# medinammartin3/Safe-Autonomous-Driving-MPC

Measured on NVIDIA B200. Metric: tracking_mpc_qp_solves_per_sec, higher is better.
Workload: dtype f64

## Files before the change

safe-autonomous-driving-mpc_b200/csrc/mpcb_api.cu:

```cuda
#include <cuda_runtime.h>
#include <math.h>
#include <stdio.h>
#include <stdlib.h>
#include <string.h>

#include <algorithm>
#include <new>
#include <type_traits>
#include <vector>

#include "mpcb200.h"
#include "mpcb_solver.cuh"
#include "mpcb_coop.cuh"

namespace mpcb {

#ifndef MPCB_SOLVE_THREADS
#define MPCB_SOLVE_THREADS 128
#endif
#ifndef MPCB_SOLVE_CTAS
#define MPCB_SOLVE_CTAS 2
#endif
#ifndef MPCB_STORE_MASK
#define MPCB_STORE_MASK 7
#endif
constexpr int SOLVE_THREADS = MPCB_SOLVE_THREADS;
using SolveStore = Store<(MPCB_STORE_MASK != 0 ? SOLVE_THREADS : 1), MPCB_STORE_MASK>;
constexpr size_t SOLVE_SMEM = sizeof(double) * SolveStore::SHARED * SOLVE_THREADS;
#ifndef MPCB_CLS_MASK0
#define MPCB_CLS_MASK0 (1u | 2u | 8u | 32u)
#endif
#ifndef MPCB_CLS_MASK1
#define MPCB_CLS_MASK1 (1u | 2u | 4u | 32u)
#endif
#ifndef MPCB_CLS_MASK2
#define MPCB_CLS_MASK2 7u
#endif
template <int NOBS> struct ClsCfg;
template <> struct ClsCfg<0> { typedef Store<SOLVE_THREADS, MPCB_CLS_MASK0, 0> St; };
template <> struct ClsCfg<1> { typedef Store<SOLVE_THREADS, MPCB_CLS_MASK1, 1> St; };
template <> struct ClsCfg<2> { typedef Store<SOLVE_THREADS, MPCB_CLS_MASK2, 2> St; };
constexpr int cmax3(int a, int b, int c) { return a > b ? (a > c ? a : c) : (b > c ? b : c); }
constexpr size_t CLS_SMEM = sizeof(double) * SOLVE_THREADS * cmax3(ClsCfg<0>::St::SHARED, ClsCfg<1>::St::SHARED, ClsCfg<2>::St::SHARED);
constexpr int CLS_HDR = 4;
constexpr int EVAL_THREADS = 128;

struct SolveIO {
  const double* x0; const double* obs_sv; const int* n_obs;
  double* U; double* Xpred; double* obj; int* status; int* iters; double* cmin; unsigned long long* active;
  double* u0;
  const int* idx;
  const int* n_idx;
  int accumulate;
  const double* U_start;
  int shift_start;
  int n_total;
};

template <bool FIRST_PASS>
__device__ __forceinline__ bool finalize(const DevTable& T, const DevParams& P, const Problem& pb, const SolveOut& so, int b,
                                         bool accumulate, const SolveIO& io, int* __restrict__ fb_list,
                                         int* __restrict__ fb_count) {
  double* __restrict__ U_out = io.U;
  double* __restrict__ Xpred_out = io.Xpred;
  double* __restrict__ obj_out = io.obj;
  int* __restrict__ status_out = io.status;
  int* __restrict__ iters_out = io.iters;
// ... 97 lines not shown
  Problem pb;
  if (live) {
#pragma unroll
    for (int c = 0; c < 5; ++c) pb.x0[c] = io.x0[(size_t)b * 5 + c];
#pragma unroll
    for (int k = 0; k < 2; ++k) { pb.obs[k][0] = io.obs_sv[(size_t)b * 4 + 2 * k]; pb.obs[k][1] = io.obs_sv[(size_t)b * 4 + 2 * k + 1]; }
    pb.n_obs = min(max(io.n_obs[b], 0), 2);
  } else {
#pragma unroll
    for (int c = 0; c < 5; ++c) pb.x0[c] = 0.0;
    pb.obs[0][0] = pb.obs[0][1] = pb.obs[1][0] = pb.obs[1][1] = 0.0;
    pb.n_obs = 0;
  }
  extern __shared__ double solve_smem[];
  double solve_local[SolveStore::LOCAL > 0 ? SolveStore::LOCAL : 1];
  const SolveStore st(solve_smem + threadIdx.x, solve_local);
  SolveOut so = solve_one<FIRST_PASS>(T, P, pb, st, live);
  if (!live) return;
  finalize<FIRST_PASS>(T, P, pb, so, b, io.accumulate != 0, io, fb_list, fb_count);
}

__global__ void __launch_bounds__(256)
mpcb_classify_kernel(int B, const int* __restrict__ idx, const int* __restrict__ n_idx, const int* __restrict__ n_obs,
                     int* __restrict__ cls) {
  const int n_work = idx ? min(*n_idx, B) : B;
  const int t = blockIdx.x * blockDim.x + threadIdx.x;
  const bool live = t < n_work;
  const int b = live ? (idx ? idx[t] : t) : 0;
  const int c = live ? min(max(n_obs[b], 0), 2) : -1;
  const unsigned lane = threadIdx.x & 31u;
#pragma unroll
  for (int k = 0; k < 3; ++k) {
    const unsigned m = __ballot_sync(0xffffffffu, c == k);
    if (m == 0u) continue;
    int base = 0;
    const int leader = __ffs(m) - 1;
    if ((int)lane == leader) base = atomicAdd(cls + k, __popc(m));
    base = __shfl_sync(0xffffffffu, base, leader);
    if (c == k) {
      const int slot = base + __popc(m & ((1u << lane) - 1u));
      MPCB_ASSERT(slot >= 0 && slot < B && b >= 0 && b < B);
      cls[CLS_HDR + (size_t)k * B + slot] = b;
    }
  }
}

__device__ __forceinline__ void load_hot_start(const SolveIO& io, int b, double (&Uh)[NV]) {
  const double* __restrict__ src = io.U_start + (size_t)b * NV;
#pragma unroll
  for (int i = 0; i < NV; ++i) Uh[i] = io.shift_start ? src[i + 2 < NV ? i + 2 : i] : src[i];
}

template <int NOBS>
__device__ __forceinline__ void solve_cls_body(const DevTable& T, const DevParams& P, const SolveIO& io, const int* __restrict__ list,
                                               int n_work, int t0, int* __restrict__ fb_list, int* __restrict__ fb_count) {
  typedef typename ClsCfg<NOBS>::St St;
  const int t = t0 + threadIdx.x;
  const bool live = t < n_work;
  const int b = live ? list[t] : 0;
  MPCB_ASSERT(b >= 0 && b < io.n_total);
  Problem pb;
  if (live) {
#pragma unroll
    for (int c = 0; c < 5; ++c) pb.x0[c] = io.x0[(size_t)b * 5 + c];
#pragma unroll
    for (int k = 0; k < 2; ++k) {
      pb.obs[k][0] = (k < NOBS) ? io.obs_sv[(size_t)b * 4 + 2 * k] : 0.0;
      pb.obs[k][1] = (k < NOBS) ? io.obs_sv[(size_t)b * 4 + 2 * k + 1] : 0.0;
    }
    pb.n_obs = NOBS;
  } else {
#pragma unroll
    for (int c = 0; c < 5; ++c) pb.x0[c] = 0.0;
    pb.obs[0][0] = pb.obs[0][1] = pb.obs[1][0] = pb.obs[1][1] = 0.0;
    pb.n_obs = 0;
  }
  extern __shared__ double solve_smem[];
  double solve_local[St::LOCAL];
  const St st(solve_smem + threadIdx.x, solve_local);
  double Uh[NV];
  const bool hot = io.U_start != nullptr;
  if (hot && live) load_hot_start(io, b, Uh);
  SolveOut so = solve_one<true>(T, P, pb, st, live, (hot && live) ? Uh : nullptr);
  if (!live) return;
  finalize<true>(T, P, pb, so, b, io.accumulate != 0, io, fb_list, fb_count);
}

__global__ void __launch_bounds__(SOLVE_THREADS, MPCB_SOLVE_CTAS)
mpcb_solve_cls_kernel(const __grid_constant__ DevTable T, const __grid_constant__ DevParams P, int B,
                      const __grid_constant__ SolveIO io, const int* __restrict__ cls, int* __restrict__ fb_list,
                      int* __restrict__ fb_count) {
  const int n2 = cls[2], n1 = cls[1], n0 = cls[0];
  const int c2 = (n2 + SOLVE_THREADS - 1) / SOLVE_THREADS, c1 = (n1 + SOLVE_THREADS - 1) / SOLVE_THREADS,
            c0 = (n0 + SOLVE_THREADS - 1) / SOLVE_THREADS;
  int blk = blockIdx.x;
  if (blk < c2) { solve_cls_body<2>(T, P, io, cls + CLS_HDR + (size_t)2 * B, n2, blk * SOLVE_THREADS, fb_list, fb_count); return; }
  blk -= c2;
  if (blk < c1) { solve_cls_body<1>(T, P, io, cls + CLS_HDR + (size_t)1 * B, n1, blk * SOLVE_THREADS, fb_list, fb_count); return; }
  blk -= c1;
  if (blk < c0) solve_cls_body<0>(T, P, io, cls + CLS_HDR, n0, blk * SOLVE_THREADS, fb_list, fb_count);
}

constexpr int COOP_WARPS = 4;
#ifndef MPCB_COOP_CTAS
#define MPCB_COOP_CTAS 2
#endif
constexpr int COOP_CTAS = MPCB_COOP_CTAS;
constexpr int FB_HDR = 4;
constexpr size_t COOP_SMEM = sizeof(WarpShared) * COOP_WARPS;

template <bool FIRST_PASS>
__global__ void __launch_bounds__(COOP_WARPS * 32, COOP_CTAS)
mpcb_coop_kernel(const __grid_constant__ DevTable T, const __grid_constant__ DevParams P, int B,
                 const __grid_constant__ SolveIO io, int* __restrict__ fb_list, int* __restrict__ fb_count,
                 int* __restrict__ cursor) {
  extern __shared__ double coop_smem[];
  const int lane = threadIdx.x & 31, wid = threadIdx.x >> 5;
  WarpShared& ws = reinterpret_cast<WarpShared*>(coop_smem)[wid];
  const int* __restrict__ idx = io.idx;
  const int n_work = idx ? min(*io.n_idx, B) : B;
  for (;;) {
    int t = 0;
    if (lane == 0) t = atomicAdd(cursor, 1);
// ... 274 lines not shown
  c->device = device;
  c->n_sm = prop.multiProcessorCount;
  c->params = *p;
  c->dp = dp;
  const int K = t->K;
  c->K = K;
  c->Ku = t->Ku;
  auto fail = [&](int code) { mpcb_destroy(c); return code; };
  if (cudaMalloc(&c->d_s, sizeof(double) * K) != cudaSuccess) return fail(cuda_fail(cudaGetLastError(), "cudaMalloc"));
  if (cudaMalloc(&c->d_y, sizeof(double) * K * 4) != cudaSuccess) return fail(cuda_fail(cudaGetLastError(), "cudaMalloc"));
  if (cudaMalloc(&c->d_u, sizeof(double) * c->Ku * 2) != cudaSuccess) return fail(cuda_fail(cudaGetLastError(), "cudaMalloc"));
  cudaError_t e;
  if ((e = cudaMemcpy(c->d_s, t->s.data(), sizeof(double) * K, cudaMemcpyHostToDevice)) != cudaSuccess) return fail(cuda_fail(e, "cudaMemcpy"));
  if ((e = cudaMemcpy(c->d_y, t->y.data(), sizeof(double) * K * 4, cudaMemcpyHostToDevice)) != cudaSuccess) return fail(cuda_fail(e, "cudaMemcpy"));
  if ((e = cudaMemcpy(c->d_u, t->u.data(), sizeof(double) * c->Ku * 2, cudaMemcpyHostToDevice)) != cudaSuccess) return fail(cuda_fail(e, "cudaMemcpy"));
  int prio_lo = 0, prio_hi = 0;
  cudaDeviceGetStreamPriorityRange(&prio_lo, &prio_hi);
  if ((e = cudaStreamCreateWithPriority(&c->stream, cudaStreamNonBlocking, prio_hi)) != cudaSuccess) return fail(cuda_fail(e, "cudaStreamCreate"));
  if ((e = cudaEventCreate(&c->ev0)) != cudaSuccess) return fail(cuda_fail(e, "cudaEventCreate"));
  if ((e = cudaEventCreate(&c->ev1)) != cudaSuccess) return fail(cuda_fail(e, "cudaEventCreate"));
  if ((e = cudaEventCreate(&c->ev_mid)) != cudaSuccess) return fail(cuda_fail(e, "cudaEventCreate"));
  if ((e = cudaEventCreateWithFlags(&c->ev_fork, cudaEventDisableTiming)) != cudaSuccess) return fail(cuda_fail(e, "cudaEventCreate"));
  if ((e = cudaFuncSetAttribute(mpcb_solve_cls_kernel, cudaFuncAttributeMaxDynamicSharedMemorySize, (int)CLS_SMEM)) != cudaSuccess ||
      (e = cudaFuncSetAttribute(mpcb_solve_kernel<false>, cudaFuncAttributeMaxDynamicSharedMemorySize, (int)SOLVE_SMEM)) != cudaSuccess ||
      (e = cudaFuncSetAttribute(mpcb_coop_kernel<true>, cudaFuncAttributeMaxDynamicSharedMemorySize, (int)COOP_SMEM)) != cudaSuccess ||
      (e = cudaFuncSetAttribute(mpcb_coop_kernel<false>, cudaFuncAttributeMaxDynamicSharedMemorySize, (int)COOP_SMEM)) != cudaSuccess)
    return fail(cuda_fail(e, "cudaFuncSetAttribute"));
  c->xs[0] = c->stream;
  for (int k = 1; k < 4; ++k) {
    if ((e = cudaStreamCreateWithPriority(&c->xs[k], cudaStreamNonBlocking, std::min(prio_lo, prio_hi + k))) != cudaSuccess) return fail(cuda_fail(e, "cudaStreamCreate"));
    if ((e = cudaEventCreateWithFlags(&c->xe[k], cudaEventDisableTiming)) != cudaSuccess) return fail(cuda_fail(e, "cudaEventCreate"));
  }
  c->dt.s = c->d_s; c->dt.y = c->d_y; c->dt.u = c->d_u;
  c->dt.K = K; c->dt.Ku = c->Ku; c->dt.s_max = t->s_max;
  {
    const int n = 4096;
    const double s0 = t->s[0], span = t->s[K - 1] - t->s[0];
    std::vector<int> lut(n);
    const double scale = span > 0 ? (double)n / span : 0.0;
    for (int b = 0; b < n; ++b) {
      const double edge = s0 + (scale > 0 ? (double)b / scale : 0.0);
      const int lo = (int)(std::lower_bound(t->s.begin(), t->s.end(), edge) - t->s.begin());
      lut[b] = std::min(std::max(lo, 1), K - 1);
    }
    if (cudaMalloc(&c->d_lut, sizeof(int) * n) != cudaSuccess) return fail(cuda_fail(cudaGetLastError(), "cudaMalloc"));
    if ((e = cudaMemcpy(c->d_lut, lut.data(), sizeof(int) * n, cudaMemcpyHostToDevice)) != cudaSuccess) return fail(cuda_fail(e, "cudaMemcpy"));
// ... 4 lines not shown
    if ((e = cudaMemcpy(c->d_sinv, sinv.data(), sizeof(double) * K, cudaMemcpyHostToDevice)) != cudaSuccess) return fail(cuda_fail(e, "cudaMemcpy"));
    c->dt.sinv = c->d_sinv;
  }
  for (int k = 0; k < 4; ++k) c->dt.last[k] = t->last_row[1 + k];
  *out = c;
  return MPCB_OK;
}

int mpcb_destroy(mpcb_handle h) {
  if (!h) return MPCB_ERR_INVALID;
  cudaSetDevice(h->device);
  if (h->d_s) cudaFree(h->d_s);
  if (h->d_y) cudaFree(h->d_y);
  if (h->d_u) cudaFree(h->d_u);
  if (h->d_lut) cudaFree(h->d_lut);
  if (h->d_sinv) cudaFree(h->d_sinv);
  for (int k = 0; k < 2; ++k) {
    if (h->gslot[k].exec) cudaGraphExecDestroy(h->gslot[k].exec);
    if (h->gslot[k].graph) cudaGraphDestroy(h->gslot[k].graph);
  }
  if (h->ev_fork) cudaEventDestroy(h->ev_fork);
  if (h->ws) cudaFree(h->ws);
  if (h->fb) cudaFree(h->fb);
  if (h->cls) cudaFree(h->cls);
  if (h->ev0) cudaEventDestroy(h->ev0);
  if (h->ev1) cudaEventDestroy(h->ev1);
  if (h->ev_mid) cudaEventDestroy(h->ev_mid);
  for (int k = 1; k < 4; ++k) {
    if (h->xs[k]) cudaStreamDestroy(h->xs[k]);
    if (h->xe[k]) cudaEventDestroy(h->xe[k]);
  }
  if (h->pin) cudaFreeHost(h->pin);
  if (h->stream) cudaStreamDestroy(h->stream);
  delete h;
  return MPCB_OK;
}

#ifndef MPCB_HOST_CHUNKS
#define MPCB_HOST_CHUNKS 4
#endif
static const int HOST_CHUNKS = MPCB_HOST_CHUNKS;
static int ensure_fb(mpcb_handle h, int B) {
  if (!h->params.fast_pass || B + FB_HDR * HOST_CHUNKS <= h->fb_cap) return MPCB_OK;
  if (h->fb) { CK(cudaFree(h->fb)); h->fb = nullptr; h->fb_cap = 0; }
  if (h->cls) { CK(cudaFree(h->cls)); h->cls = nullptr; }
  if (cudaMalloc(&h->fb, sizeof(int) * ((size_t)B + FB_HDR * HOST_CHUNKS)) != cudaSuccess) { cudaGetLastError(); return MPCB_ERR_NOMEM; }
  if (cudaMalloc(&h->cls, sizeof(int) * 3 * ((size_t)B + FB_HDR * HOST_CHUNKS)) != cudaSuccess) { cudaGetLastError(); return MPCB_ERR_NOMEM; }
  h->fb_cap = B + FB_HDR * HOST_CHUNKS;
  return MPCB_OK;
}

static cudaError_t record_event(cudaEvent_t ev, cudaStream_t st) {
  cudaStreamCaptureStatus cs = cudaStreamCaptureStatusNone;
  cudaError_t e = cudaStreamIsCapturing(st, &cs);
  if (e != cudaSuccess) return e;
  return cudaEventRecordWithFlags(ev, st, cs == cudaStreamCaptureStatusActive ? cudaEventRecordExternal : cudaEventRecordDefault);
}

static bool call_uses_coop(mpcb_handle h, int B_total) { return h->params.fast_pass && B_total <= h->params.coop_max_batch; }

static int launch_solve(mpcb_handle h, int B, const SolveIO& io_in, cudaStream_t st, int* fb, bool timed, bool use_coop,
                        bool part = false) {
  const int grid = (B + SOLVE_THREADS - 1) / SOLVE_THREADS;
  SolveIO io = io_in;
  io.n_total = B;
  h->last_shape = (h->params.fast_pass && use_coop) ? 1 : 0;
  if (timed) CK(record_event(h->ev0, st));
  if (h->params.fast_pass) {
    int* fb_count = fb;
    int* fb_list = fb + FB_HDR;
    CK(cudaMemsetAsync(fb, 0, sizeof(int) * FB_HDR, st));
    if (use_coop) {
      const int g1 = std::min((B + COOP_WARPS - 1) / COOP_WARPS, h->n_sm * COOP_CTAS);
      mpcb_coop_kernel<true><<<g1, COOP_WARPS * 32, COOP_SMEM, st>>>(h->dt, h->dp, B, io, fb_list, fb_count, fb + 1);
    } else {
      int* cls = h->cls + (fb - h->fb) * 3;
      CK(cudaMemsetAsync(cls, 0, sizeof(int) * CLS_HDR, st));
      mpcb_classify_kernel<<<(B + 255) / 256, 256, 0, st>>>(B, io.idx, io.n_idx, io.n_obs, cls);
      CK(cudaGetLastError());
      SolveIO io1 = io;
      io1.idx = nullptr; io1.n_idx = nullptr;
      mpcb_solve_cls_kernel<<<grid + 2, SOLVE_THREADS, CLS_SMEM, st>>>(h->dt, h->dp, B, io1, cls, fb_list, fb_count);
      h->launches++;
    }
    CK(cudaGetLastError());
    if (timed) CK(record_event(h->ev_mid, st));
    SolveIO io2 = io;
    io2.idx = fb_list;
    io2.n_idx = fb_count;
    io2.accumulate = 1;
    if (h->params.coop_pass2) {
      const int full = std::min(h->n_sm * COOP_CTAS, (B + COOP_WARPS - 1) / COOP_WARPS);
      const int g2 = (part && !use_coop) ? std::min(full, std::max(16, (B + 63) / 64)) : full;
      mpcb_coop_kernel<false><<<g2, COOP_WARPS * 32, COOP_SMEM, st>>>(h->dt, h->dp, B, io2, nullptr, nullptr, fb + 2);
    } else {
      const int t2 = (MPCB_STORE_MASK == 0) ? 32 : SOLVE_THREADS;
      mpcb_solve_kernel<false><<<(B + t2 - 1) / t2, t2, SOLVE_SMEM, st>>>(h->dt, h->dp, B, io2, nullptr, nullptr);
    }
    CK(cudaGetLastError());
    h->launches += 2;
  } else {
    if (timed) CK(record_event(h->ev_mid, st));
    mpcb_solve_kernel<false><<<grid, SOLVE_THREADS, SOLVE_SMEM, st>>>(h->dt, h->dp, B, io, nullptr, nullptr);
    CK(cudaGetLastError());
    h->launches++;
  }
// ... 20 lines not shown
                     double* Xpred_out, double* obj_out, int* status_out, int* iters_out, double* cmin_out,
                     unsigned long long* active_out, void* cuda_stream) {
  if (!h || B < 0 || (B > 0 && (!x0 || !obs_sv || !n_obs || !U_out))) return MPCB_ERR_INVALID;
  if ((((size_t)U_out) | ((size_t)Xpred_out)) & 15u) return MPCB_ERR_INVALID;
  if (B == 0) return MPCB_OK;
  CK(cudaSetDevice(h->device));
  int rc = ensure_fb(h, B);
  if (rc != MPCB_OK) return rc;
  return launch_solve(h, B, make_io(x0, obs_sv, n_obs, U_out, Xpred_out, obj_out, status_out, iters_out, cmin_out, active_out),
                      (cudaStream_t)cuda_stream, h->fb, true, call_uses_coop(h, B));
}

int mpcb_solve_list_internal(mpcb_handle h, int B, const int* idx, const int* n_idx, const double* x0, const double* obs_sv,
                             const int* n_obs, double* U_out, int* status_out, cudaStream_t st, const double* U_start) {
  int rc = ensure_fb(h, B);
  if (rc != MPCB_OK) return rc;
  SolveIO io = make_io(x0, obs_sv, n_obs, U_out, nullptr, nullptr, status_out, nullptr, nullptr, nullptr);
  io.idx = idx;
  io.n_idx = n_idx;
  io.U_start = U_start;
  io.shift_start = 1;
  return launch_solve(h, B, io, st, h->fb, true, call_uses_coop(h, B));
}

static size_t al256(size_t x) { return (x + 255) & ~(size_t)255; }

static double part_edge(int c) {
  static double edges[17];
  static bool init = false;
  if (!init) {
    for (int k = 0; k <= HOST_CHUNKS; ++k) edges[k] = (double)k / HOST_CHUNKS;
    if (HOST_CHUNKS == 4) { edges[1] = 0.125; edges[2] = 0.375; edges[3] = 0.6875; }
#ifdef MPCB_DEV
    if (const char* e = getenv("MPCB_HOST_SPLIT")) {
      int k = 1;
      while (*e && k < HOST_CHUNKS) { edges[k++] = atof(e); while (*e && *e != ',') ++e; if (*e == ',') ++e; }
    }
#endif
    init = true;
  }
  return edges[c];
}

static const int HOST_PACKED_MAX = 2048;

static int solve_host(mpcb_handle h, int B, const double* x0, const double* obs_sv, const int* n_obs,
                      double* U_out, double* Xpred_out, double* obj_out, int* status_out, int* iters_out,
                      double* cmin_out, unsigned long long* active_out, double* u0_out, bool wait = true) {
// ... 17 lines not shown
  double* dX = Xpred_out ? (double*)(w + o_X) : nullptr;
  double* dobj = obj_out ? (double*)(w + o_obj) : nullptr;
  int* dst = status_out ? (int*)(w + o_st) : nullptr;
  int* dit = iters_out ? (int*)(w + o_it) : nullptr;
  double* dcm = cmin_out ? (double*)(w + o_cm) : nullptr;
  unsigned long long* dac = active_out ? (unsigned long long*)(w + o_ac) : nullptr;
  double* du0 = u0_out ? (double*)(w + o_u0) : nullptr;
  const bool use_coop = call_uses_coop(h, B);

  const bool packed = B <= HOST_PACKED_MAX;
  if (packed && total > h->pin_bytes) {
    if (h->pin) { cudaFreeHost(h->pin); h->pin = nullptr; h->pin_bytes = 0; }
    size_t want = total;
    { const size_t nmax = HOST_PACKED_MAX; want = std::max(want, (size_t)(al256(nmax * 40) + al256(nmax * 32) + 2 * al256(nmax * 4) + al256(nmax * 80) + al256(nmax * 240) + 4 * al256(nmax * 8) + al256(nmax * 16))); }
    if (cudaHostAlloc(&h->pin, want, cudaHostAllocDefault) != cudaSuccess) { cudaGetLastError(); return MPCB_ERR_NOMEM; }
    h->pin_bytes = want;
  }
  mpcb_ctx::GraphSlot& g = h->gslot[packed ? 0 : 1];
  const void* up[11] = {x0, obs_sv, n_obs, U_out, Xpred_out, obj_out, status_out, iters_out, cmin_out, active_out, u0_out};
  unsigned long long key[16] = {(unsigned long long)B, (unsigned long long)(size_t)h->ws, (unsigned long long)(size_t)h->fb,
                                (unsigned long long)(size_t)h->pin, 0, 0, 0, 0, 0, 0, 0, 0, 0, 0, 0, 0};
  for (int k = 3; k < 11; ++k) key[4] |= (unsigned long long)(up[k] != nullptr) << k;
  key[4] |= (unsigned long long)(wait ? 0 : 1) << 32;
  if (!packed)
    for (int k = 0; k < 11; ++k) key[5 + k] = (unsigned long long)(size_t)up[k];
  const bool hit = g.valid && memcmp(g.key, key, sizeof(key)) == 0;
  bool capture = false;
  if (!hit) {
    capture = g.have_last && memcmp(g.last, key, sizeof(key)) == 0;
#ifdef MPCB_DEV
    if (getenv("MPCB_NO_GRAPH")) capture = false;
#endif
    if (capture && !packed) {
      for (int k = 0; k < 11 && capture; ++k) {
        if (!up[k]) continue;
        cudaPointerAttributes at;
        if (cudaPointerGetAttributes(&at, up[k]) != cudaSuccess || at.type != cudaMemoryTypeHost) { cudaGetLastError(); capture = false; }
      }
    }
    memcpy(g.last, key, sizeof(key));
    g.have_last = true;
  }
  cudaStream_t s0 = h->xs[0];

  auto enqueue = [&]() -> int {
    if (packed) {
// ... 193 lines not shown
  CK(cudaEventElapsedTime(&b, h->ev_mid, h->ev1));
  if (first_ms) *first_ms = a;
  if (second_ms) *second_ms = b;
  if (n_second) {
    *n_second = 0;
    if (h->params.fast_pass && h->fb_last) CK(cudaMemcpy(n_second, h->fb_last, sizeof(int), cudaMemcpyDeviceToHost));
  }
  return MPCB_OK;
}

#ifdef MPCB_COOP_PROFILE
int mpcb_debug_coop_profile(unsigned long long* sum8, unsigned long long* max8, int reset) {
  if (sum8) CK(cudaMemcpyFromSymbol(sum8, g_coop_sum, 64));
  if (max8) CK(cudaMemcpyFromSymbol(max8, g_coop_max, 64));
  if (reset) {
    unsigned long long z[8] = {0, 0, 0, 0, 0, 0, 0, 0};
    CK(cudaMemcpyToSymbol(g_coop_sum, z, 64));
    CK(cudaMemcpyToSymbol(g_coop_max, z, 64));
  }
  return MPCB_OK;
}
#endif

unsigned long long mpcb_launch_count(mpcb_handle h) { return h ? h->launches : 0ull; }
int mpcb_last_first_pass_shape(mpcb_handle h) { return h ? h->last_shape : MPCB_ERR_INVALID; }

int mpcb_measure_fp64_peak(mpcb_handle h, double* tflops, float* ms_out) {
  if (!h || !tflops) return MPCB_ERR_INVALID;
  CK(cudaSetDevice(h->device));
  cudaDeviceProp prop;
  CK(cudaGetDeviceProperties(&prop, h->device));
  const int blocks = prop.multiProcessorCount * 8, threads = 256, iters = 4096;
  double* d = nullptr;
  CK(cudaMalloc(&d, sizeof(double) * blocks * threads));
  cudaStream_t st = h->stream;
  float best = 1e30f;
  for (int rep = 0; rep < 5; ++rep) {
    cudaEventRecord(h->ev0, st);
    mpcb_dfma_probe<<<blocks, threads, 0, st>>>(d, iters, 0.999999, 1e-7);
    cudaEventRecord(h->ev1, st);
    cudaError_t e = cudaStreamSynchronize(st);
    if (e != cudaSuccess) { cudaFree(d); return cuda_fail(e, "dfma probe"); }
    float ms = 0;
    cudaEventElapsedTime(&ms, h->ev0, h->ev1);
    if (rep > 0) best = std::min(best, ms);
    h->launches++;
// ... 11 lines not shown
```

safe-autonomous-driving-mpc_b200/csrc/mpcb_internal.h:

```cpp
#pragma once
#include <cuda_runtime.h>
#include <stdio.h>

#include "mpcb200.h"
#include "mpcb_device.cuh"

extern thread_local char g_cuda_err[512];
int cuda_fail(cudaError_t e, const char* where);

#define CK(call)                                        \
  do {                                                  \
    cudaError_t e_ = (call);                            \
    if (e_ != cudaSuccess) return cuda_fail(e_, #call); \
  } while (0)

struct mpcb_ctx {
  int device;
  int n_sm = 148;
  mpcb_params params;
  mpcb::DevParams dp;
  mpcb::DevTable dt;
  int K, Ku;
  double* d_s = nullptr;
  double* d_y = nullptr;
  double* d_u = nullptr;
  int* d_lut = nullptr;
  double* d_sinv = nullptr;
  void* ws = nullptr;
  size_t ws_bytes = 0;
  int* fb = nullptr;
  int fb_cap = 0;
  int* cls = nullptr;
  cudaStream_t stream = nullptr;
  cudaEvent_t ev0 = nullptr, ev1 = nullptr, ev_mid = nullptr;
  cudaStream_t xs[4] = {nullptr, nullptr, nullptr, nullptr};
  cudaEvent_t xe[4] = {nullptr, nullptr, nullptr, nullptr};
  void* pin = nullptr;
  size_t pin_bytes = 0;
  int* fb_last = nullptr;
  bool timed = false;
  bool pass_timed = false;
  int last_shape = 0;
  unsigned long long launches = 0;
  struct GraphSlot {
    bool valid = false, have_last = false;
    unsigned long long key[16] = {0}, last[16] = {0};
    cudaGraph_t graph = nullptr;
    cudaGraphExec_t exec = nullptr;
    unsigned long long launches = 0;
  } gslot[2];
  cudaEvent_t ev_fork = nullptr;
};

extern "C" int mpcb_solve_list_internal(mpcb_handle h, int B, const int* idx, const int* n_idx, const double* x0,
                                        const double* obs_sv, const int* n_obs, double* U_out, int* status_out,
// ... 2 lines not shown
```

safe-autonomous-driving-mpc_b200/csrc/mpcb_solver.cuh:

```cuda
#pragma once
#include <type_traits>

#include "mpcb200.h"
#include "mpcb_device.cuh"

#if defined(__CUDA_ARCH__) && defined(MPCB_WARP_UNIFORM)
#define MPCB_ALL(pred) (__all_sync(0xffffffffu, pred) != 0)
#elif defined(__CUDA_ARCH__)
#define MPCB_ALL(pred) (__syncthreads_and(pred) != 0)
#else
#define MPCB_ALL(pred) (pred)
#endif

namespace mpcb {

constexpr int N_LANE = 8;
constexpr int ROW_LANE = 10, ROW_V = 18, ROW_OBS = 23, N_OBSROW = 9, M_ROWS = 41;
constexpr int N_DO = 20;
constexpr double NRM2_FLOOR = 1e-2;

__host__ __device__ constexpr int doff(int jj) { return jj * (jj + 1); }
__host__ __device__ constexpr int row_r1(int k, int j) { return ROW_OBS + N_OBSROW * k + (j - 2); }
__host__ __device__ constexpr int row_r2(int k, int j) { return ROW_OBS + N_OBSROW * k + 4 + (j - 1); }

// ... 552 lines not shown
#pragma unroll
    for (int k = 0; k < 2; ++k) {
      if (k < ST::KOBS) {
        const double base = (pb.obs[k][0] + pb.obs[k][1] * (j * P.h)) - pb.x0[0] - j * P.h * pb.x0[4];
        const bool on = k < pb.n_obs;
        if (j > 1) st.hio[N_OBSROW * k + (j - 2)] = (!on || dead_1[k][j - 1]) ? BIG : base - P.obs_safe;
        st.hio[N_OBSROW * k + 4 + (j - 1)] = (!on || dead_2[k][j - 1]) ? BIG : base - P.tgap * pb.x0[4];
        screened |= on && (dead_1[k][j - 1] || dead_2[k][j - 1]);
      }
    }
  }
#pragma unroll
  for (int i = 0; i < NH; ++i) { st.blo[i] = blo[i]; st.bhi[i] = bhi[i]; }
  if (ur) warm_fill(P, pb.x0, pb.obs, pb.n_obs, ur, pb.U);
  else warm_start(T, P, pb.x0, pb.obs, pb.n_obs, pb.U, pb.hint);
  pb.hint[NH] = pb.hint[NH - 1];
#pragma unroll
  for (int i = 0; i < NV; ++i) pb.U[i] = clipd(pb.U[i], P.umin[i & 1], P.umax[i & 1]);
#pragma unroll
  for (int i = 0; i < NH; ++i) pb.U[2 * i + 1] = clipd(pb.U[2 * i + 1], blo[i], bhi[i]);
  return screened;
}

template <bool FIRST_PASS, class ST>
MPCB_HD SolveOut solve_one(const DevTable& T, const DevParams& P, Problem& pb, const ST& st, bool live,
                           const double* U_start = nullptr) {
  SolveOut out{MPCB_MAXITER, 0, 0, false};
  const bool screened = prologue(T, P, pb, st);
  const bool hot = FIRST_PASS && U_start != nullptr;
  if (U_start) {
#pragma unroll
    for (int i = 0; i < NV; ++i) {
      const double u = clipd(U_start[i], P.umin[i & 1], P.umax[i & 1]);
      pb.U[i] = (i & 1) ? clipd(u, st.blo[i >> 1], st.bhi[i >> 1]) : u;
    }
  }
  bool done = !live;
  bool infeasible = screened;
  out.const_infeasible = screened;
  bool first = true;
  const Policy& pl = P.pol[FIRST_PASS ? 1 : 0];
  double step_prev = 1e30;
  int fails = 0;
  const int max_rounds = FIRST_PASS ? P.thread_max_rounds : P.max_rounds;
  const int max_segments = FIRST_PASS ? P.thread_max_segments : pl.max_segments;
  auto cold_start = [&](const double (&xx)[NV]) {
#pragma unroll
    for (int i = 0; i < 6; ++i) pb.E.w[i] = 0x11111111u * (unsigned)pl.e_init;
    unsigned long long act0 = 0ull;
    for_rows(P, pb, st, xx, [&](int r, double zt, double lo, double hi, auto kind) {
      constexpr int KIND = decltype(kind)::value;
      st.v[r] = clipk<KIND>(zt, lo, hi);
      if (hot) {
        const bool at_lo = (KIND != 2) && (zt <= lo + P.feas_tol), at_hi = (KIND != 1) && (zt >= hi - P.feas_tol);
        if (at_lo || at_hi) act0 |= (1ull << r);
      }
    });
    pb.act_prev = act0;
  };
  for (int round = 0; round < max_rounds; ++round) {
    if (MPCB_ALL(done)) break;
    if (!done) {
      double cviol;
      linearise(T, P, pb, st, cviol);
      if (first) {
        cold_start(pb.U);
#pragma unroll
        for (int i = 0; i < NV; ++i) pb.x[i] = pb.U[i];
        first = false;
      }
      if (cviol > P.feas_tol) { infeasible = true; out.const_infeasible = true; }
      out.rounds++;
    }
    const double loosen = (FIRST_PASS || P.qp_forcing <= 0.0) ? 1.0
                          : dmax(1.0, (step_prev * P.qp_forcing < P.qp_eps_loose ? step_prev * P.qp_forcing : P.qp_eps_loose) / P.eps_p);
    const double eps_p = P.eps_p * loosen, eps_d = P.eps_d * loosen;
    bool conv = false;
    bool qdone = done;
    bool cert = false;
    for (int seg = 0; seg < max_segments; ++seg) {
      if (MPCB_ALL(qdone)) break;
      if (!qdone) {
        factor<FIRST_PASS>(P, pl, pb, st);
        SegStats s;
        for (int it = 0; it < pl.segment_iters - 1; ++it) admm_iter<false, false, FIRST_PASS>(P, pl, pb, st, s);
        admm_iter<true, !FIRST_PASS, FIRST_PASS>(P, pl, pb, st, s, eps_p);
        out.iters += pl.segment_iters;
#ifdef MPCB_TRACE
        if (getenv("MPCB_TRACE")) {
          printf("  r%d s%d pass %d rp %.2e rd %.2e nd %.2e act %011llx E", round, seg, FIRST_PASS ? 1 : 2, s.rp, s.rd, s.nd, pb.act_prev);
          for (int r = 0; r < M_ROWS; ++r) printf("%d", pb.E.get(r));
          printf(" x");
          for (int i = 0; i < NV; ++i) printf(" %.4f", pb.x[i]);
          printf("\n");
        }
#endif
        if (s.rp <= eps_p && s.rd <= eps_d) { conv = true; qdone = true; }
        else if (!FIRST_PASS && s.nd > 1e-9 && s.atdy <= P.eps_inf * s.nd && s.sup < -P.eps_inf * s.nd &&
                 s.bad <= P.eps_inf * s.nd) { conv = true; cert = true; qdone = true; }
      }
    }
    if (!done) {
      double step = 0.0;
#pragma unroll
      for (int i = 0; i < NV; ++i) { step = dmax(step, fabs(pb.x[i] - pb.U[i])); pb.U[i] = pb.x[i]; }
      step_prev = step;
      if (cert) { infeasible = true; done = true; }
      else if (conv && step < P.step_tol) { done = true; out.status = 0; }
      else if (!conv) {
        ++fails;
        if (FIRST_PASS ? fails > P.fast_fail_rounds : fails >= P.max_fail_rounds) done = true;
      }
    }
  }
  if (infeasible && (!FIRST_PASS || out.status == 0)) out.status = 2;
#pragma unroll
  for (int i = 0; i < NV; ++i) pb.U[i] = clipd(pb.U[i], P.umin[i & 1], P.umax[i & 1]);
  return out;
}

}
```

Baseline: 163.5 million.

## Compact unconverged problems between SQP rounds via parked state and per-round kernels

Splits the per-thread solve into start/round/end phases. After a few initial rounds, problems that have not converged have their solver state written to a global carry buffer and are compacted by warp-level atomics. Later rounds each run as a separate kernel that processes only the still-active problems. This targets warp divergence and idle lanes from problems that finish early, at the cost of extra kernel launches and global round-trips of per-problem state. Compaction is only enabled when the grid exceeds one wave of resident CTAs.

```diff
diff --git a/safe-autonomous-driving-mpc_b200/csrc/mpcb_api.cu b/safe-autonomous-driving-mpc_b200/csrc/mpcb_api.cu
--- a/safe-autonomous-driving-mpc_b200/csrc/mpcb_api.cu
+++ b/safe-autonomous-driving-mpc_b200/csrc/mpcb_api.cu
@@ -43,6 +43,7 @@
 constexpr int cmax3(int a, int b, int c) { return a > b ? (a > c ? a : c) : (b > c ? b : c); }
 constexpr size_t CLS_SMEM = sizeof(double) * SOLVE_THREADS * cmax3(ClsCfg<0>::St::SHARED, ClsCfg<1>::St::SHARED, ClsCfg<2>::St::SHARED);
 constexpr int CLS_HDR = 4;
+constexpr int CARRY_HDR = 12;
 constexpr int EVAL_THREADS = 128;
 
 struct SolveIO {
@@ -186,7 +187,8 @@
 
 __global__ void __launch_bounds__(256)
 mpcb_classify_kernel(int B, const int* __restrict__ idx, const int* __restrict__ n_idx, const int* __restrict__ n_obs,
-                     int* __restrict__ cls) {
+                     int* __restrict__ cls, int* __restrict__ carry_hdr) {
+  if (blockIdx.x == 0 && threadIdx.x < CARRY_HDR) carry_hdr[threadIdx.x] = 0;
   const int n_work = idx ? min(*n_idx, B) : B;
   const int t = blockIdx.x * blockDim.x + threadIdx.x;
   const bool live = t < n_work;
@@ -215,54 +217,224 @@
   for (int i = 0; i < NV; ++i) Uh[i] = io.shift_start ? src[i + 2 < NV ? i + 2 : i] : src[i];
 }
 
+#ifndef MPCB_CLS_ROUNDS
+#define MPCB_CLS_ROUNDS 4
+#endif
+constexpr int CLS_ROUNDS = MPCB_CLS_ROUNDS;
+
+enum : int { CD_U = 0, CD_X = CD_U + NV, CD_V = CD_X + NV, CD_LOV = CD_V + ROW_OBS + 2 * N_OBSROW, CD_BLO = CD_LOV + NH,
+             CD_BHI = CD_BLO + NH, CD_HIO = CD_BHI + NH, N_CD = CD_HIO + 2 * N_OBSROW };
+enum : int { CI_B = 0, CI_HINT = 1, CI_FAILS = CI_HINT + NH + 1, CI_ROUNDS, CI_ITERS, CI_STATUS, CI_FLAGS, N_CI };
+constexpr size_t CARRY_SLOT_BYTES = sizeof(double) * N_CD + sizeof(unsigned long long) + sizeof(int) * N_CI;
+
+struct Carry {
+  double* d; unsigned long long* a; int* i; int cap;
+  __host__ __device__ static Carry at(void* base, int cap) {
+    Carry c;
+    c.d = (double*)base;
+    c.a = (unsigned long long*)(c.d + (size_t)N_CD * cap);
+    c.i = (int*)(c.a + cap);
+    c.cap = cap;
+    return c;
+  }
+};
+
+__device__ __forceinline__ int warp_append(bool pred, int* counter) {
+  const unsigned m = __ballot_sync(0xffffffffu, pred);
+  if (m == 0u) return -1;
+  const unsigned lane = threadIdx.x & 31u;
+  const int leader = __ffs(m) - 1;
+  int base = 0;
+  if ((int)lane == leader) base = atomicAdd(counter, __popc(m));
+  base = __shfl_sync(0xffffffffu, base, leader);
+  return pred ? base + __popc(m & ((1u << lane) - 1u)) : -1;
+}
+
+template <class ST>
+__device__ __forceinline__ void park(const Carry& c, int slot, int b, const Problem& pb, const ST& st, const SolveState& s) {
+  MPCB_ASSERT(slot >= 0 && slot < c.cap);
+  double* __restrict__ d = c.d + slot;
+  int* __restrict__ iv = c.i + slot;
+  const size_t n = c.cap;
+#pragma unroll
+  for (int k = 0; k < NV; ++k) { d[(CD_U + k) * n] = pb.U[k]; d[(CD_X + k) * n] = pb.x[k]; }
+#pragma unroll
+  for (int r = 0; r < ST::MROWS; ++r) d[(CD_V + r) * n] = st.v[r];
+#pragma unroll
+  for (int j = 0; j < NH; ++j) { d[(CD_LOV + j) * n] = st.lov[j]; d[(CD_BLO + j) * n] = st.blo[j]; d[(CD_BHI + j) * n] = st.bhi[j]; }
+#pragma unroll
+  for (int r = 0; r < ST::KOBS * N_OBSROW; ++r) d[(CD_HIO + r) * n] = st.hio[r];
+  c.a[slot] = pb.act_prev;
+  iv[CI_B * n] = b;
+#pragma unroll
+  for (int j = 0; j <= NH; ++j) iv[(CI_HINT + j) * n] = pb.hint[j];
+  iv[CI_FAILS * n] = s.fails;
+  iv[CI_ROUNDS * n] = s.out.rounds;
+  iv[CI_ITERS * n] = s.out.iters;
+  iv[CI_STATUS * n] = s.out.status;
+  iv[CI_FLAGS * n] = (s.infeasible ? 1 : 0) | (s.out.const_infeasible ? 2 : 0);
+}
+
+template <class ST>
+__device__ __forceinline__ void unpark(const Carry& c, int slot, Problem& pb, const ST& st, SolveState& s) {
+  MPCB_ASSERT(slot >= 0 && slot < c.cap);
+  const double* __restrict__ d = c.d + slot;
+  const int* __restrict__ iv = c.i + slot;
+  const size_t n = c.cap;
+#pragma unroll
+  for (int k = 0; k < NV; ++k) { pb.U[k] = d[(CD_U + k) * n]; pb.x[k] = d[(CD_X + k) * n]; }
+#pragma unroll
+  for (int r = 0; r < ST::MROWS; ++r) st.v[r] = d[(CD_V + r) * n];
+#pragma unroll
+  for (int j = 0; j < NH; ++j) { st.lov[j] = d[(CD_LOV + j) * n]; st.blo[j] = d[(CD_BLO + j) * n]; st.bhi[j] = d[(CD_BHI + j) * n]; }
+#pragma unroll
+  for (int r = 0; r < ST::KOBS * N_OBSROW; ++r) st.hio[r] = d[(CD_HIO + r) * n];
+  pb.act_prev = c.a[slot];
+#pragma unroll
+  for (int j = 0; j <= NH; ++j) pb.hint[j] = iv[(CI_HINT + j) * n];
+  s.fails = iv[CI_FAILS * n];
+  s.out.rounds = iv[CI_ROUNDS * n];
+  s.out.iters = iv[CI_ITERS * n];
+  s.out.status = iv[CI_STATUS * n];
+  const int f = iv[CI_FLAGS * n];
+  s.infeasible = (f & 1) != 0;
+  s.out.const_infeasible = (f & 2) != 0;
+  s.done = false; s.first = false; s.hot = false;
+  s.step_prev = 1e30;
+}
+
+template <int NOBS>
+__device__ __forceinline__ void load_problem(const SolveIO& io, int b, bool live, Problem& pb) {
+  if (live) {
+#pragma unroll
+    for (int c = 0; c < 5; ++c) pb.x0[c] = io.x0[(size_t)b * 5 + c];
+#pragma unroll
+    for (int k = 0; k < 2; ++k) {
+      pb.obs[k][0] = (k < NOBS) ? io.obs_sv[(size_t)b * 4 + 2 * k] : 0.0;
+      pb.obs[k][1] = (k < NOBS) ? io.obs_sv[(size_t)b * 4 + 2 * k + 1] : 0.0;
+    }
+    pb.n_obs = NOBS;
+  } else {
+#pragma unroll
+    for (int c = 0; c < 5; ++c) pb.x0[c] = 0.0;
+    pb.obs[0][0] = pb.obs[0][1] = pb.obs[1][0] = pb.obs[1][1] = 0.0;
+    pb.n_obs = 0;
+  }
+}
+
+template <int NOBS, class ST>
+__device__ __forceinline__ void park_or_finalize(const DevTable& T, const DevParams& P, const SolveIO& io, bool live, bool cont,
+                                                 int b, Problem& pb, const ST& st, SolveState& s, int n_work,
+                                                 const Carry& cout, int* __restrict__ cnt_out, int off,
+                                                 int* __restrict__ fb_list, int* __restrict__ fb_count) {
+  const int k = warp_append(cont, cnt_out + NOBS);
+  if (!live) return;
+  if (cont) {
+    MPCB_ASSERT(k >= 0 && k < n_work);
+    park(cout, off + k, b, pb, st, s);
+    return;
+  }
+  const SolveOut so = solve_end<true>(P, pb, s);
+  finalize<true>(T, P, pb, so, b, io.accumulate != 0, io, fb_list, fb_count);
+}
+
 template <int NOBS>
 __device__ __forceinline__ void solve_cls_body(const DevTable& T, const DevParams& P, const SolveIO& io, const int* __restrict__ list,
-                                               int n_work, int t0, int* __restrict__ fb_list, int* __restrict__ fb_count) {
+                                               int n_work, int t0, int off, int r0, const Carry& cout,
+                                               int* __restrict__ cnt_out, int* __restrict__ fb_list, int* __restrict__ fb_count) {
   typedef typename ClsCfg<NOBS>::St St;
   const int t = t0 + threadIdx.x;
   const bool live = t < n_work;
   const int b = live ? list[t] : 0;
   MPCB_ASSERT(b >= 0 && b < io.n_total);
   Problem pb;
-  if (live) {
-#pragma unroll
-    for (int c = 0; c < 5; ++c) pb.x0[c] = io.x0[(size_t)b * 5 + c];
-#pragma unroll
-    for (int k = 0; k < 2; ++k) {
-      pb.obs[k][0] = (k < NOBS) ? io.obs_sv[(size_t)b * 4 + 2 * k] : 0.0;
-      pb.obs[k][1] = (k < NOBS) ? io.obs_sv[(size_t)b * 4 + 2 * k + 1] : 0.0;
-    }
-    pb.n_obs = NOBS;
-  } else {
-#pragma unroll
-    for (int c = 0; c < 5; ++c) pb.x0[c] = 0.0;
-    pb.obs[0][0] = pb.obs[0][1] = pb.obs[1][0] = pb.obs[1][1] = 0.0;
-    pb.n_obs = 0;
-  }
+  load_problem<NOBS>(io, b, live, pb);
   extern __shared__ double solve_smem[];
   double solve_local[St::LOCAL];
   const St st(solve_smem + threadIdx.x, solve_local);
   double Uh[NV];
   const bool hot = io.U_start != nullptr;
   if (hot && live) load_hot_start(io, b, Uh);
-  SolveOut so = solve_one<true>(T, P, pb, st, live, (hot && live) ? Uh : nullptr);
-  if (!live) return;
-  finalize<true>(T, P, pb, so, b, io.accumulate != 0, io, fb_list, fb_count);
+  SolveState s;
+  solve_start<true>(T, P, pb, st, live, (hot && live) ? Uh : nullptr, s);
+#pragma unroll 1
+  for (int round = 0; round < r0; ++round) {
+    if (MPCB_ALL(s.done)) break;
+    solve_round<true>(T, P, pb, st, s, round);
+  }
+  park_or_finalize<NOBS>(T, P, io, live, live && !s.done && r0 < P.thread_max_rounds, b, pb, st, s, n_work, cout, cnt_out,
+                         off, fb_list, fb_count);
+}
+
+__device__ __forceinline__ int class_offset(const int* __restrict__ cls, int k) {
+  return k == 2 ? 0 : (k == 1 ? cls[2] : cls[2] + cls[1]);
 }
 
 __global__ void __launch_bounds__(SOLVE_THREADS, MPCB_SOLVE_CTAS)
 mpcb_solve_cls_kernel(const __grid_constant__ DevTable T, const __grid_constant__ DevParams P, int B,
-                      const __grid_constant__ SolveIO io, const int* __restrict__ cls, int* __restrict__ fb_list,
+                      const __grid_constant__ SolveIO io, const int* __restrict__ cls, int r0,
+                      const __grid_constant__ Carry cout, int* __restrict__ cnt_out, int* __restrict__ fb_list,
                       int* __restrict__ fb_count) {
   const int n2 = cls[2], n1 = cls[1], n0 = cls[0];
   const int c2 = (n2 + SOLVE_THREADS - 1) / SOLVE_THREADS, c1 = (n1 + SOLVE_THREADS - 1) / SOLVE_THREADS,
             c0 = (n0 + SOLVE_THREADS - 1) / SOLVE_THREADS;
+  const int* lists = cls + CLS_HDR;
   int blk = blockIdx.x;
-  if (blk < c2) { solve_cls_body<2>(T, P, io, cls + CLS_HDR + (size_t)2 * B, n2, blk * SOLVE_THREADS, fb_list, fb_count); return; }
+  if (blk < c2) { solve_cls_body<2>(T, P, io, lists + (size_t)2 * B, n2, blk * SOLVE_THREADS, 0, r0, cout, cnt_out, fb_list, fb_count); return; }
   blk -= c2;
-  if (blk < c1) { solve_cls_body<1>(T, P, io, cls + CLS_HDR + (size_t)1 * B, n1, blk * SOLVE_THREADS, fb_list, fb_count); return; }
+  if (blk < c1) { solve_cls_body<1>(T, P, io, lists + (size_t)1 * B, n1, blk * SOLVE_THREADS, n2, r0, cout, cnt_out, fb_list, fb_count); return; }
   blk -= c1;
-  if (blk < c0) solve_cls_body<0>(T, P, io, cls + CLS_HDR, n0, blk * SOLVE_THREADS, fb_list, fb_count);
+  if (blk < c0) solve_cls_body<0>(T, P, io, lists, n0, blk * SOLVE_THREADS, n2 + n1, r0, cout, cnt_out, fb_list, fb_count);
+}
+
+#ifdef MPCB_ROUND_STATS
+__device__ unsigned long long g_round_stats[16 * 3];
+#endif
+
+template <int NOBS>
+__device__ __forceinline__ void solve_round_body(const DevTable& T, const DevParams& P, const SolveIO& io, int n_work, int t0,
+                                                 int off, const Carry& cin, const Carry& cout, int* __restrict__ cnt_out,
+                                                 int round, int* __restrict__ fb_list, int* __restrict__ fb_count) {
+  typedef typename ClsCfg<NOBS>::St St;
+  const int t = t0 + threadIdx.x;
+  const bool live = t < n_work;
+  const int slot = off + t;
+  MPCB_ASSERT(!live || (slot >= 0 && slot < cin.cap));
+  const int b = live ? cin.i[(size_t)CI_B * cin.cap + slot] : 0;
+  MPCB_ASSERT(b >= 0 && b < io.n_total);
+  Problem pb;
+  load_problem<NOBS>(io, b, live, pb);
+  extern __shared__ double solve_smem[];
+  double solve_local[St::LOCAL];
+  const St st(solve_smem + threadIdx.x, solve_local);
+  SolveState s;
+  s.out = SolveOut{MPCB_MAXITER, 0, 0, false};
+  s.done = true; s.infeasible = false; s.first = false; s.hot = false; s.fails = 0; s.step_prev = 1e30;
+  if (live) unpark(cin, slot, pb, st, s);
+  solve_round<true>(T, P, pb, st, s, round);
+  park_or_finalize<NOBS>(T, P, io, live, live && !s.done && round + 1 < P.thread_max_rounds, b, pb, st, s, n_work, cout,
+                         cnt_out, off, fb_list, fb_count);
+}
+
+__global__ void __launch_bounds__(SOLVE_THREADS, MPCB_SOLVE_CTAS)
+mpcb_solve_round_kernel(const __grid_constant__ DevTable T, const __grid_constant__ DevParams P,
+                        const __grid_constant__ SolveIO io, const int* __restrict__ cls, const int* __restrict__ cnt_in,
+                        const __grid_constant__ Carry cin, int* __restrict__ cnt_out, const __grid_constant__ Carry cout,
+                        int* __restrict__ cnt_clear, int round, int* __restrict__ fb_list, int* __restrict__ fb_count) {
+  if (blockIdx.x == 0 && threadIdx.x < 3) cnt_clear[threadIdx.x] = 0;
+  const int n2 = cnt_in[2], n1 = cnt_in[1], n0 = cnt_in[0];
+#ifdef MPCB_ROUND_STATS
+  if (blockIdx.x == 0 && threadIdx.x < 3 && round < 16) atomicAdd(&g_round_stats[3 * round + threadIdx.x], (unsigned long long)cnt_in[threadIdx.x]);
+#endif
+  MPCB_ASSERT(n2 >= 0 && n2 <= cls[2] && n1 >= 0 && n1 <= cls[1] && n0 >= 0 && n0 <= cls[0]);
+  const int c2 = (n2 + SOLVE_THREADS - 1) / SOLVE_THREADS, c1 = (n1 + SOLVE_THREADS - 1) / SOLVE_THREADS,
+            c0 = (n0 + SOLVE_THREADS - 1) / SOLVE_THREADS;
+  int blk = blockIdx.x;
+  if (blk < c2) { solve_round_body<2>(T, P, io, n2, blk * SOLVE_THREADS, class_offset(cls, 2), cin, cout, cnt_out, round, fb_list, fb_count); return; }
+  blk -= c2;
+  if (blk < c1) { solve_round_body<1>(T, P, io, n1, blk * SOLVE_THREADS, class_offset(cls, 1), cin, cout, cnt_out, round, fb_list, fb_count); return; }
+  blk -= c1;
+  if (blk < c0) solve_round_body<0>(T, P, io, n0, blk * SOLVE_THREADS, class_offset(cls, 0), cin, cout, cnt_out, round, fb_list, fb_count);
 }
 
 constexpr int COOP_WARPS = 4;
@@ -583,6 +755,7 @@
   if ((e = cudaEventCreate(&c->ev_mid)) != cudaSuccess) return fail(cuda_fail(e, "cudaEventCreate"));
   if ((e = cudaEventCreateWithFlags(&c->ev_fork, cudaEventDisableTiming)) != cudaSuccess) return fail(cuda_fail(e, "cudaEventCreate"));
   if ((e = cudaFuncSetAttribute(mpcb_solve_cls_kernel, cudaFuncAttributeMaxDynamicSharedMemorySize, (int)CLS_SMEM)) != cudaSuccess ||
+      (e = cudaFuncSetAttribute(mpcb_solve_round_kernel, cudaFuncAttributeMaxDynamicSharedMemorySize, (int)CLS_SMEM)) != cudaSuccess ||
       (e = cudaFuncSetAttribute(mpcb_solve_kernel<false>, cudaFuncAttributeMaxDynamicSharedMemorySize, (int)SOLVE_SMEM)) != cudaSuccess ||
       (e = cudaFuncSetAttribute(mpcb_coop_kernel<true>, cudaFuncAttributeMaxDynamicSharedMemorySize, (int)COOP_SMEM)) != cudaSuccess ||
       (e = cudaFuncSetAttribute(mpcb_coop_kernel<false>, cudaFuncAttributeMaxDynamicSharedMemorySize, (int)COOP_SMEM)) != cudaSuccess)
@@ -633,7 +806,6 @@
   if (h->ev_fork) cudaEventDestroy(h->ev_fork);
   if (h->ws) cudaFree(h->ws);
   if (h->fb) cudaFree(h->fb);
-  if (h->cls) cudaFree(h->cls);
   if (h->ev0) cudaEventDestroy(h->ev0);
   if (h->ev1) cudaEventDestroy(h->ev1);
   if (h->ev_mid) cudaEventDestroy(h->ev_mid);
@@ -651,13 +823,19 @@
 #define MPCB_HOST_CHUNKS 4
 #endif
 static const int HOST_CHUNKS = MPCB_HOST_CHUNKS;
+static size_t al256(size_t x) { return (x + 255) & ~(size_t)255; }
+
 static int ensure_fb(mpcb_handle h, int B) {
   if (!h->params.fast_pass || B + FB_HDR * HOST_CHUNKS <= h->fb_cap) return MPCB_OK;
-  if (h->fb) { CK(cudaFree(h->fb)); h->fb = nullptr; h->fb_cap = 0; }
-  if (h->cls) { CK(cudaFree(h->cls)); h->cls = nullptr; }
-  if (cudaMalloc(&h->fb, sizeof(int) * ((size_t)B + FB_HDR * HOST_CHUNKS)) != cudaSuccess) { cudaGetLastError(); return MPCB_ERR_NOMEM; }
-  if (cudaMalloc(&h->cls, sizeof(int) * 3 * ((size_t)B + FB_HDR * HOST_CHUNKS)) != cudaSuccess) { cudaGetLastError(); return MPCB_ERR_NOMEM; }
-  h->fb_cap = B + FB_HDR * HOST_CHUNKS;
+  if (h->fb) { CK(cudaFree(h->fb)); h->fb = nullptr; h->cls = nullptr; h->carry = nullptr; h->fb_cap = 0; }
+  const size_t cap = (size_t)B + FB_HDR * HOST_CHUNKS;
+  const size_t o_cls = al256(sizeof(int) * cap), o_carry = o_cls + al256(sizeof(int) * 3 * cap);
+  void* p = nullptr;
+  if (cudaMalloc(&p, o_carry + 2 * cap * CARRY_SLOT_BYTES) != cudaSuccess) { cudaGetLastError(); return MPCB_ERR_NOMEM; }
+  h->fb = (int*)p;
+  h->cls = (int*)((char*)p + o_cls);
+  h->carry = (char*)p + o_carry;
+  h->fb_cap = (int)cap;
   return MPCB_OK;
 }
 
@@ -686,13 +864,28 @@
       mpcb_coop_kernel<true><<<g1, COOP_WARPS * 32, COOP_SMEM, st>>>(h->dt, h->dp, B, io, fb_list, fb_count, fb + 1);
     } else {
       int* cls = h->cls + (fb - h->fb) * 3;
+      char* cw = h->carry + (size_t)(fb - h->fb) * 2 * CARRY_SLOT_BYTES;
+      int* hdr = (int*)cw;
+      const size_t w0 = FB_HDR * 2 * CARRY_SLOT_BYTES;
+      const Carry wk[2] = {Carry::at(cw + w0, B), Carry::at(cw + w0 + (size_t)B * CARRY_SLOT_BYTES, B)};
       CK(cudaMemsetAsync(cls, 0, sizeof(int) * CLS_HDR, st));
-      mpcb_classify_kernel<<<(B + 255) / 256, 256, 0, st>>>(B, io.idx, io.n_idx, io.n_obs, cls);
+      mpcb_classify_kernel<<<(B + 255) / 256, 256, 0, st>>>(B, io.idx, io.n_idx, io.n_obs, cls, hdr);
       CK(cudaGetLastError());
       SolveIO io1 = io;
       io1.idx = nullptr; io1.n_idx = nullptr;
-      mpcb_solve_cls_kernel<<<grid + 2, SOLVE_THREADS, CLS_SMEM, st>>>(h->dt, h->dp, B, io1, cls, fb_list, fb_count);
+      const int max_rounds = h->dp.thread_max_rounds;
+      const bool compact = grid > h->n_sm * MPCB_SOLVE_CTAS;
+      const int r0 = compact ? std::min(CLS_ROUNDS, max_rounds) : max_rounds;
+      mpcb_solve_cls_kernel<<<grid + 2, SOLVE_THREADS, CLS_SMEM, st>>>(h->dt, h->dp, B, io1, cls, r0, wk[0],
+                                                                      hdr + 4 * (r0 % 3), fb_list, fb_count);
       h->launches++;
+      for (int r = r0; r < max_rounds; ++r) {
+        const int p = (r - r0) & 1;
+        mpcb_solve_round_kernel<<<grid + 2, SOLVE_THREADS, CLS_SMEM, st>>>(h->dt, h->dp, io1, cls, hdr + 4 * (r % 3), wk[p],
+                                                                          hdr + 4 * ((r + 1) % 3), wk[p ^ 1],
+                                                                          hdr + 4 * ((r + 2) % 3), r, fb_list, fb_count);
+        h->launches++;
+      }
     }
     CK(cudaGetLastError());
     if (timed) CK(record_event(h->ev_mid, st));
@@ -759,8 +952,6 @@
   io.shift_start = 1;
   return launch_solve(h, B, io, st, h->fb, true, call_uses_coop(h, B));
 }
-
-static size_t al256(size_t x) { return (x + 255) & ~(size_t)255; }
 
 static double part_edge(int c) {
   static double edges[17];
@@ -824,6 +1015,7 @@
                                 (unsigned long long)(size_t)h->pin, 0, 0, 0, 0, 0, 0, 0, 0, 0, 0, 0, 0};
   for (int k = 3; k < 11; ++k) key[4] |= (unsigned long long)(up[k] != nullptr) << k;
   key[4] |= (unsigned long long)(wait ? 0 : 1) << 32;
+  key[4] |= (unsigned long long)h->fb_cap << 33;
   if (!packed)
     for (int k = 0; k < 11; ++k) key[5 + k] = (unsigned long long)(size_t)up[k];
   const bool hit = g.valid && memcmp(g.key, key, sizeof(key)) == 0;
@@ -1063,6 +1255,17 @@
 }
 #endif
 
+#ifdef MPCB_ROUND_STATS
+int mpcb_debug_round_counts(unsigned long long* counts48, int reset) {
+  if (counts48) CK(cudaMemcpyFromSymbol(counts48, g_round_stats, sizeof(unsigned long long) * 48));
+  if (reset) {
+    unsigned long long z[48] = {0};
+    CK(cudaMemcpyToSymbol(g_round_stats, z, sizeof(z)));
+  }
+  return MPCB_OK;
+}
+#endif
+
 unsigned long long mpcb_launch_count(mpcb_handle h) { return h ? h->launches : 0ull; }
 int mpcb_last_first_pass_shape(mpcb_handle h) { return h ? h->last_shape : MPCB_ERR_INVALID; }
 
diff --git a/safe-autonomous-driving-mpc_b200/csrc/mpcb_internal.h b/safe-autonomous-driving-mpc_b200/csrc/mpcb_internal.h
--- a/safe-autonomous-driving-mpc_b200/csrc/mpcb_internal.h
+++ b/safe-autonomous-driving-mpc_b200/csrc/mpcb_internal.h
@@ -31,6 +31,7 @@
   int* fb = nullptr;
   int fb_cap = 0;
   int* cls = nullptr;
+  char* carry = nullptr;
   cudaStream_t stream = nullptr;
   cudaEvent_t ev0 = nullptr, ev1 = nullptr, ev_mid = nullptr;
   cudaStream_t xs[4] = {nullptr, nullptr, nullptr, nullptr};
diff --git a/safe-autonomous-driving-mpc_b200/csrc/mpcb_solver.cuh b/safe-autonomous-driving-mpc_b200/csrc/mpcb_solver.cuh
--- a/safe-autonomous-driving-mpc_b200/csrc/mpcb_solver.cuh
+++ b/safe-autonomous-driving-mpc_b200/csrc/mpcb_solver.cuh
@@ -598,12 +598,19 @@
   return screened;
 }
 
+struct SolveState {
+  SolveOut out;
+  bool done, infeasible, first, hot;
+  int fails;
+  double step_prev;
+};
+
 template <bool FIRST_PASS, class ST>
-MPCB_HD SolveOut solve_one(const DevTable& T, const DevParams& P, Problem& pb, const ST& st, bool live,
-                           const double* U_start = nullptr) {
-  SolveOut out{MPCB_MAXITER, 0, 0, false};
+MPCB_HD void solve_start(const DevTable& T, const DevParams& P, Problem& pb, const ST& st, bool live,
+                         const double* U_start, SolveState& s) {
+  s.out = SolveOut{MPCB_MAXITER, 0, 0, false};
   const bool screened = prologue(T, P, pb, st);
-  const bool hot = FIRST_PASS && U_start != nullptr;
+  s.hot = FIRST_PASS && U_start != nullptr;
   if (U_start) {
 #pragma unroll
     for (int i = 0; i < NV; ++i) {
@@ -611,15 +618,19 @@
       pb.U[i] = (i & 1) ? clipd(u, st.blo[i >> 1], st.bhi[i >> 1]) : u;
     }
   }
-  bool done = !live;
-  bool infeasible = screened;
-  out.const_infeasible = screened;
-  bool first = true;
+  s.done = !live;
+  s.infeasible = screened;
+  s.out.const_infeasible = screened;
+  s.first = true;
+  s.step_prev = 1e30;
+  s.fails = 0;
+}
+
+template <bool FIRST_PASS, class ST>
+MPCB_HD void solve_round(const DevTable& T, const DevParams& P, Problem& pb, const ST& st, SolveState& s, int round) {
   const Policy& pl = P.pol[FIRST_PASS ? 1 : 0];
-  double step_prev = 1e30;
-  int fails = 0;
-  const int max_rounds = FIRST_PASS ? P.thread_max_rounds : P.max_rounds;
   const int max_segments = FIRST_PASS ? P.thread_max_segments : pl.max_segments;
+  const bool hot = s.hot;
   auto cold_start = [&](const double (&xx)[NV]) {
 #pragma unroll
     for (int i = 0; i < 6; ++i) pb.E.w[i] = 0x11111111u * (unsigned)pl.e_init;
@@ -634,65 +645,82 @@
     });
     pb.act_prev = act0;
   };
-  for (int round = 0; round < max_rounds; ++round) {
-    if (MPCB_ALL(done)) break;
-    if (!done) {
-      double cviol;
-      linearise(T, P, pb, st, cviol);
-      if (first) {
-        cold_start(pb.U);
-#pragma unroll
-        for (int i = 0; i < NV; ++i) pb.x[i] = pb.U[i];
-        first = false;
-      }
-      if (cviol > P.feas_tol) { infeasible = true; out.const_infeasible = true; }
-      out.rounds++;
-    }
-    const double loosen = (FIRST_PASS || P.qp_forcing <= 0.0) ? 1.0
-                          : dmax(1.0, (step_prev * P.qp_forcing < P.qp_eps_loose ? step_prev * P.qp_forcing : P.qp_eps_loose) / P.eps_p);
-    const double eps_p = P.eps_p * loosen, eps_d = P.eps_d * loosen;
-    bool conv = false;
-    bool qdone = done;
-    bool cert = false;
-    for (int seg = 0; seg < max_segments; ++seg) {
-      if (MPCB_ALL(qdone)) break;
-      if (!qdone) {
-        factor<FIRST_PASS>(P, pl, pb, st);
-        SegStats s;
-        for (int it = 0; it < pl.segment_iters - 1; ++it) admm_iter<false, false, FIRST_PASS>(P, pl, pb, st, s);
-        admm_iter<true, !FIRST_PASS, FIRST_PASS>(P, pl, pb, st, s, eps_p);
-        out.iters += pl.segment_iters;
+  if (!s.done) {
+    double cviol;
+    linearise(T, P, pb, st, cviol);
+    if (s.first) {
+      cold_start(pb.U);
+#pragma unroll
+      for (int i = 0; i < NV; ++i) pb.x[i] = pb.U[i];
+      s.first = false;
+    }
+    if (cviol > P.feas_tol) { s.infeasible = true; s.out.const_infeasible = true; }
+    s.out.rounds++;
+  }
+  const double step_prev = s.step_prev;
+  const double loosen = (FIRST_PASS || P.qp_forcing <= 0.0) ? 1.0
+                        : dmax(1.0, (step_prev * P.qp_forcing < P.qp_eps_loose ? step_prev * P.qp_forcing : P.qp_eps_loose) / P.eps_p);
+  const double eps_p = P.eps_p * loosen, eps_d = P.eps_d * loosen;
+  bool conv = false;
+  bool qdone = s.done;
+  bool cert = false;
+  for (int seg = 0; seg < max_segments; ++seg) {
+    if (MPCB_ALL(qdone)) break;
+    if (!qdone) {
+      factor<FIRST_PASS>(P, pl, pb, st);
+      SegStats ss;
+      for (int it = 0; it < pl.segment_iters - 1; ++it) admm_iter<false, false, FIRST_PASS>(P, pl, pb, st, ss);
+      admm_iter<true, !FIRST_PASS, FIRST_PASS>(P, pl, pb, st, ss, eps_p);
+      s.out.iters += pl.segment_iters;
 #ifdef MPCB_TRACE
-        if (getenv("MPCB_TRACE")) {
-          printf("  r%d s%d pass %d rp %.2e rd %.2e nd %.2e act %011llx E", round, seg, FIRST_PASS ? 1 : 2, s.rp, s.rd, s.nd, pb.act_prev);
-          for (int r = 0; r < M_ROWS; ++r) printf("%d", pb.E.get(r));
-          printf(" x");
-          for (int i = 0; i < NV; ++i) printf(" %.4f", pb.x[i]);
-          printf("\n");
-        }
+      if (getenv("MPCB_TRACE")) {
+        printf("  r%d s%d pass %d rp %.2e rd %.2e nd %.2e act %011llx E", round, seg, FIRST_PASS ? 1 : 2, ss.rp, ss.rd, ss.nd, pb.act_prev);
+        for (int r = 0; r < M_ROWS; ++r) printf("%d", pb.E.get(r));
+        printf(" x");
+        for (int i = 0; i < NV; ++i) printf(" %.4f", pb.x[i]);
+        printf("\n");
+      }
 #endif
-        if (s.rp <= eps_p && s.rd <= eps_d) { conv = true; qdone = true; }
-        else if (!FIRST_PASS && s.nd > 1e-9 && s.atdy <= P.eps_inf * s.nd && s.sup < -P.eps_inf * s.nd &&
-                 s.bad <= P.eps_inf * s.nd) { conv = true; cert = true; qdone = true; }
-      }
-    }
-    if (!done) {
-      double step = 0.0;
-#pragma unroll
-      for (int i = 0; i < NV; ++i) { step = dmax(step, fabs(pb.x[i] - pb.U[i])); pb.U[i] = pb.x[i]; }
-      step_prev = step;
-      if (cert) { infeasible = true; done = true; }
-      else if (conv && step < P.step_tol) { done = true; out.status = 0; }
-      else if (!conv) {
-        ++fails;
-        if (FIRST_PASS ? fails > P.fast_fail_rounds : fails >= P.max_fail_rounds) done = true;
-      }
-    }
-  }
-  if (infeasible && (!FIRST_PASS || out.status == 0)) out.status = 2;
+      if (ss.rp <= eps_p && ss.rd <= eps_d) { conv = true; qdone = true; }
+      else if (!FIRST_PASS && ss.nd > 1e-9 && ss.atdy <= P.eps_inf * ss.nd && ss.sup < -P.eps_inf * ss.nd &&
+               ss.bad <= P.eps_inf * ss.nd) { conv = true; cert = true; qdone = true; }
+    }
+  }
+  (void)round;
+  if (!s.done) {
+    double step = 0.0;
+#pragma unroll
+    for (int i = 0; i < NV; ++i) { step = dmax(step, fabs(pb.x[i] - pb.U[i])); pb.U[i] = pb.x[i]; }
+    s.step_prev = step;
+    if (cert) { s.infeasible = true; s.done = true; }
+    else if (conv && step < P.step_tol) { s.done = true; s.out.status = 0; }
+    else if (!conv) {
+      ++s.fails;
+      if (FIRST_PASS ? s.fails > P.fast_fail_rounds : s.fails >= P.max_fail_rounds) s.done = true;
+    }
+  }
+}
+
+template <bool FIRST_PASS>
+MPCB_HD SolveOut solve_end(const DevParams& P, Problem& pb, const SolveState& s) {
+  SolveOut out = s.out;
+  if (s.infeasible && (!FIRST_PASS || out.status == 0)) out.status = 2;
 #pragma unroll
   for (int i = 0; i < NV; ++i) pb.U[i] = clipd(pb.U[i], P.umin[i & 1], P.umax[i & 1]);
   return out;
 }
 
-}
+template <bool FIRST_PASS, class ST>
+MPCB_HD SolveOut solve_one(const DevTable& T, const DevParams& P, Problem& pb, const ST& st, bool live,
+                           const double* U_start = nullptr) {
+  SolveState s;
+  solve_start<FIRST_PASS>(T, P, pb, st, live, U_start, s);
+  const int max_rounds = FIRST_PASS ? P.thread_max_rounds : P.max_rounds;
+  for (int round = 0; round < max_rounds; ++round) {
+    if (MPCB_ALL(s.done)) break;
+    solve_round<FIRST_PASS>(T, P, pb, st, s, round);
+  }
+  return solve_end<FIRST_PASS>(P, pb, s);
+}
+
+}
```

Measured after the change: 177.7 million, median of 6. +8.6%, better.
